# hannesweisbach/channelcoding

Measured on AMD Instinct MI355X. Metric: decoded frames/sec (coded bits/sec = value x 255), BCH(255,231) min-sum, batch=2^20, higher is better.
Workload: dtype f32

## Files before the change

### channelcoding_amd/csrc/cc_internal.hpp

```cpp
#pragma once
#include <hip/hip_runtime.h>

#include <cstdint>
#include <memory>
#include <mutex>
#include <string>
#include <vector>

#include "../../include/channelcoding_amd.h"
#include "galois.hpp"

namespace ccamd {

struct MinSumGeometry {
  int W = 64, C = 4, frames_per_wave = 1, KW = 1;
};

struct MinSumParams {
  int n, K, KW;
  int variant;
  int stop_rule;
  unsigned iterations;
  float alpha_f;
  float beta_f;
  double beta_d;
  const uint32_t *colmask;
  float *gstate;
  unsigned long long gslab;
  uint32_t *ctl = nullptr;
  unsigned sample = 0;
  uint32_t *list = nullptr;
  unsigned list_cap = 0;
  int gate = -1;
  int first_pass = 0;
  int dual = 0;
  const float *llr2 = nullptr;
  uint8_t *hard2 = nullptr;
  uint16_t *iters2 = nullptr;
  int32_t *status2 = nullptr;
};

#if defined(__HIPCC__)
__device__ __forceinline__ bool two_pass_sampled(const MinSumParams &p) { return p.ctl[2] * 8u < p.sample; }
__device__ __forceinline__ bool two_pass_in_effect(const uint32_t *ctl, unsigned sample, unsigned cap) {
  return ctl[2] * 8u < sample && ctl[3] == 0u && ctl[1] <= cap;
}
#endif

struct AlgebraicTables {
  uint8_t exp[512];
  uint8_t log[512];
  uint8_t g[256];
  uint8_t roots_log[64];
  int n, k, l, t, nroots, family, q;
};

struct WideTables {
  const uint16_t *exp = nullptr, *log = nullptr;
  const uint16_t *g = nullptr;
  uint32_t root_log[64] = {0};
  uint32_t n = 0, k = 0, l = 0, t = 0, nroots = 0, q = 0;
  int family = 0;
};

}

namespace ccamd {
struct McWorkspace;
void mc_workspace_free(McWorkspace *w);
struct HostStage;
void host_stage_free(HostStage *s);
}

struct cc_code {
  cc_desc desc;
  int device = 0;
  std::unique_ptr<ccamd::Field> field;
  ccamd::CodeTables tab;
  bool wide = false;
  std::unique_ptr<ccamd::FieldT<uint16_t>> field16;
  ccamd::CodeTablesT<uint16_t> tab16;
  ccamd::WideTables wide_dev;
  uint16_t *d_wide = nullptr;
  bool soft = false;
  std::vector<uint8_t> custom_H;
  bool matrix_only = false;
  unsigned ms_rows = 0;
  ccamd::MinSumGeometry geo;
  uint32_t *d_colmask = nullptr;
  uint16_t *d_diag = nullptr;
  uint32_t *d_colbits = nullptr;
  uint8_t *d_parity = nullptr;
  ccamd::AlgebraicTables *d_alg = nullptr;
  ccamd::AlgebraicTables h_alg;
  mutable ccamd::McWorkspace *mc = nullptr;
  mutable ccamd::HostStage *stage = nullptr;
  mutable std::mutex lazy_lock;
  hipMemPool_t pool = nullptr;
  int num_cus = 256;
  bool force_generic = false;
  std::string name;
};

namespace ccamd {

inline hipError_t workspace_alloc(const cc_code *code, void **p, size_t bytes, hipStream_t stream) {
  return code->pool ? hipMallocFromPoolAsync(p, bytes, code->pool, stream) : hipMallocAsync(p, bytes, stream);
}

void set_last_error(const std::string &s);
int hip_fail(hipError_t e, const char *what);

#define CC_HIP_TRY(expr)                                   \
  do {                                                     \
    hipError_t _e = (expr);                                \
    if (_e != hipSuccess) return ccamd::hip_fail(_e, #expr); \
  } while (0)

int launch_minsum(const cc_code *code, const float *d_llr, const uint16_t *d_er, const uint32_t *d_er_off,
                  uint8_t *d_hard, float *d_L, uint16_t *d_iters, int32_t *d_status, size_t B, hipStream_t stream);
struct DiagGeometry {
  unsigned n, k, w;
  int D, LPF, CPL;
  bool scms;
  int np = 0;
  int gap[4] = {0, 0, 0, 0};
};
const DiagGeometry *diag_geometry(const CodeTables &t);
std::vector<uint16_t> build_diag_table(const CodeTables &t, int D, int W, int np = 0, const int *gap = nullptr);
size_t minsum_diag_lds_bytes(const DiagGeometry &g);
MinSumParams minsum_params(const cc_code *code);
bool minsum_shortcuts_enabled();
bool minsum_diag_supported(const cc_code *code);
int launch_minsum_diag_compact(const cc_code *code, uint32_t *d_ctl, unsigned cap, const float *d_llr, uint8_t *d_hard,
                               uint16_t *d_iters, int32_t *d_status, hipStream_t stream);
std::string minsum_diag_name(const cc_code *code);
int launch_minsum_diag(const cc_code *code, const MinSumParams &p, const float *d_llr, const uint16_t *d_er,
                       const uint32_t *d_er_off, uint8_t *d_hard, float *d_L, uint16_t *d_iters, int32_t *d_status,
                       size_t B, hipStream_t stream);
bool algebraic_long_needed(const cc_code *code, bool erasures);
int launch_algebraic_long(const cc_code *code, bool float_in, const void *d_in, const uint16_t *d_er,
                          const uint32_t *d_er_off, uint8_t *d_out, int32_t *d_nerr, int32_t *d_status, size_t B,
                          hipStream_t stream);
int launch_algebraic(const cc_code *code, bool float_in, const void *d_in, const uint16_t *d_er,
                     const uint32_t *d_er_off, uint8_t *d_out, int32_t *d_nerr, int32_t *d_status, size_t B,
                     hipStream_t stream);
bool algebraic_chunk_supported(const cc_code *code, bool erasures);
int launch_algebraic_chunk(const cc_code *code, bool float_in, const void *d_in, const uint16_t *d_er,
                           const uint32_t *d_er_off, uint8_t *d_out, int32_t *d_nerr, int32_t *d_status, size_t B,
                           hipStream_t stream);
bool bitslice_supported(const cc_code *code);
int launch_bitslice_syndromes(const cc_code *code, bool float_in, const void *d_in, uint8_t *d_out, uint8_t *d_synd, size_t B,
                              hipStream_t stream);
bool bitslice_encode_supported(const cc_code *code);
int launch_bitslice_encode(const cc_code *code, const uint8_t *d_msg, uint8_t *d_cw, size_t B, hipStream_t stream);
int launch_pgz_erasures(const cc_code *code, const uint8_t *d_in, const uint16_t *d_er, const uint32_t *d_er_off,
                        uint8_t *d_out, int32_t *d_nerr, int32_t *d_status, size_t B, hipStream_t stream);
constexpr int diag_variant_part(int variant, int parts) {
  const int order = variant == CC_ALG_MS ? 0 : variant == CC_ALG_NMS ? 1 : variant == CC_ALG_OMS ? 2
                  : variant == CC_ALG_SCMS2 ? 3 : variant == CC_ALG_SCMS1 ? 4 : 5;
  return order % parts;
}

int launch_wide_correct(const cc_code *code, const uint16_t *d_in, const uint16_t *d_er, const uint32_t *d_off,
                        uint16_t *d_out, int32_t *d_nerr, int32_t *d_status, size_t B, hipStream_t stream);
int launch_wide_pgz_erasures(const cc_code *code, const uint16_t *d_in, const uint16_t *d_er, const uint32_t *d_off,
                        uint16_t *d_out, int32_t *d_nerr, int32_t *d_status, size_t B, hipStream_t stream);
int launch_wide_encode(const cc_code *code, const uint16_t *d_msg, uint16_t *d_cw, size_t B, hipStream_t stream);
int launch_wide_extract(const cc_code *code, const uint16_t *d_cw, uint16_t *d_msg, size_t B, hipStream_t stream);
std::vector<uint8_t> build_parity_table(const Field &f, const CodeTables &t);
int launch_encode(const cc_code *code, const uint8_t *d_msg, uint8_t *d_cw, size_t B, hipStream_t stream);
int launch_encode_bits(const cc_code *code, const uint8_t *d_msg, uint8_t *d_cw, size_t B, hipStream_t stream);
int launch_extract(const cc_code *code, const uint8_t *d_cw, uint8_t *d_msg, size_t B, hipStream_t stream);
int mc_run(cc_code *code, double ebno_db, uint64_t seed, uint64_t first_frame, size_t frames, int random_codewords,
           uint64_t *d_counters, hipStream_t stream);
int mc_awgn(cc_code *code, double ebno_db, uint64_t seed, uint64_t first_frame, size_t frames, int random_codewords,
            float *d_llr, uint8_t *d_sent, hipStream_t stream);
int minsum_kernel_info(const cc_code *code, std::string &name, uint32_t &frames_per_wg, uint32_t &threads,
                       uint32_t &lds);

}
```

### channelcoding_amd/csrc/mc.hip

```cpp
#include <cmath>
#include <mutex>

#include "cc_internal.hpp"
#include "wave_ops.hpp"

namespace ccamd {
namespace {

struct Philox {
  uint32_t c[4];
};

__device__ __forceinline__ Philox philox4x32_10(uint32_t c0, uint32_t c1, uint32_t c2, uint32_t c3, uint32_t k0,
                                                uint32_t k1) {
  constexpr uint32_t M0 = 0xD2511F53u, M1 = 0xCD9E8D57u, W0 = 0x9E3779B9u, W1 = 0xBB67AE85u;
#pragma unroll
  for (int r = 0; r < 10; ++r) {
    const uint64_t p0 = static_cast<uint64_t>(M0) * c0, p1 = static_cast<uint64_t>(M1) * c2;
    const uint32_t hi0 = static_cast<uint32_t>(p0 >> 32), lo0 = static_cast<uint32_t>(p0);
    const uint32_t hi1 = static_cast<uint32_t>(p1 >> 32), lo1 = static_cast<uint32_t>(p1);
    const uint32_t n0 = hi1 ^ c1 ^ k0, n1 = lo1, n2 = hi0 ^ c3 ^ k1, n3 = lo0;
    c0 = n0;
    c1 = n1;
    c2 = n2;
// ... 262 lines not shown

}

struct McWorkspace {
  std::mutex lock;
  size_t chunk = 0;
  float *llr = nullptr;
  uint8_t *sent = nullptr, *msg = nullptr, *hard = nullptr;
  uint16_t *iters = nullptr;
  int32_t *status = nullptr, *nerr = nullptr;
  uint32_t *list = nullptr;
  hipEvent_t done = nullptr;
  int fence_in(hipStream_t stream) {
    if (done) CC_HIP_TRY(hipStreamWaitEvent(stream, done, 0));
    return CC_OK;
  }
  int fence_out(hipStream_t stream) {
    if (!done) CC_HIP_TRY(hipEventCreateWithFlags(&done, hipEventDisableTiming));
    CC_HIP_TRY(hipEventRecord(done, stream));
    return CC_OK;
  }
  ~McWorkspace() {
    if (done) (void)hipEventDestroy(done);
    for (void *p : {static_cast<void *>(llr), static_cast<void *>(sent), static_cast<void *>(msg),
                    static_cast<void *>(hard), static_cast<void *>(iters), static_cast<void *>(status),
                    static_cast<void *>(nerr), static_cast<void *>(list)})
      if (p) (void)hipFree(p);
  }
};

void mc_workspace_free(McWorkspace *w) { delete w; }

static int ensure_workspace(cc_code *code, size_t chunk) {
  if (!code->mc) code->mc = new McWorkspace();
  McWorkspace &w = *code->mc;
  if (w.chunk >= chunk) return CC_OK;
  const size_t n = code->tab.n, l = code->tab.l;
  for (void **p : {reinterpret_cast<void **>(&w.llr), reinterpret_cast<void **>(&w.sent),
                   reinterpret_cast<void **>(&w.msg), reinterpret_cast<void **>(&w.hard),
                   reinterpret_cast<void **>(&w.iters), reinterpret_cast<void **>(&w.status),
                   reinterpret_cast<void **>(&w.nerr), reinterpret_cast<void **>(&w.list)})
    if (*p) {
      (void)hipFree(*p);
      *p = nullptr;
    }
  w.chunk = 0;
  CC_HIP_TRY(hipMalloc(reinterpret_cast<void **>(&w.llr), chunk * n * sizeof(float)));
  CC_HIP_TRY(hipMalloc(reinterpret_cast<void **>(&w.sent), chunk * n));
  CC_HIP_TRY(hipMalloc(reinterpret_cast<void **>(&w.msg), chunk * l));
  CC_HIP_TRY(hipMalloc(reinterpret_cast<void **>(&w.hard), chunk * n));
  CC_HIP_TRY(hipMalloc(reinterpret_cast<void **>(&w.iters), chunk * sizeof(uint16_t)));
  CC_HIP_TRY(hipMalloc(reinterpret_cast<void **>(&w.status), chunk * sizeof(int32_t)));
  CC_HIP_TRY(hipMalloc(reinterpret_cast<void **>(&w.nerr), chunk * sizeof(int32_t)));
  CC_HIP_TRY(hipMalloc(reinterpret_cast<void **>(&w.list), (chunk + 64) * sizeof(uint32_t)));
  w.chunk = chunk;
  return CC_OK;
}

static int launch_sent_words(const cc_code *code, uint64_t seed, uint64_t first_frame, size_t frames, uint8_t *d_sent,
                             uint8_t *d_msg_scratch, hipStream_t stream) {
  if (!d_sent || !d_msg_scratch) return CC_ERR_INVALID_ARGUMENT;
  const int l = static_cast<int>(code->tab.l);
  const uint32_t k0 = static_cast<uint32_t>(seed), k1 = static_cast<uint32_t>(seed >> 32);
  int bits_log2 = 0;
  while ((16 << bits_log2) < l) ++bits_log2;
  const unsigned long long items = static_cast<unsigned long long>(frames) << bits_log2;
  hipLaunchKernelGGL(random_bits_kernel, dim3(grid_for(code, items)), dim3(256), 0, stream, d_msg_scratch, l, bits_log2,
                     static_cast<unsigned long long>(first_frame), static_cast<unsigned long long>(frames), k0, k1);
  return launch_encode_bits(code, d_msg_scratch, d_sent, frames, stream);
}

static bool mc_precheck_pays(const cc_code *code, double ebno_db) {
  if (!code->soft || code->d_colbits == nullptr || !minsum_diag_supported(code) || code->force_generic) return false;
  if (!minsum_shortcuts_enabled()) return false;
  const unsigned n = code->tab.n;
  if (n <= 128 || n > 256) return false;
  const int alg = code->desc.algorithm;
  const bool scaled = alg == CC_ALG_NMS || alg == CC_ALG_2DNMS;
  if (scaled && !(code->desc.alpha > 0.0)) return false;
  const double sigma = cc_sigma(code, ebno_db);
  const double pbit = 0.5 * std::erfc(1.0 / (sigma * std::sqrt(2.0)));
  return std::pow(1.0 - pbit, static_cast<double>(n)) >= 0.25;
}

int launch_awgn(const cc_code *code, double ebno_db, uint64_t seed, uint64_t first_frame, size_t frames,
                int random_codewords, float *d_llr, uint8_t *d_sent, uint8_t *d_msg_scratch, hipStream_t stream,
                unsigned long long *d_counters = nullptr, bool hard_bytes = false) {
  if (frames == 0) return CC_OK;
  const int n = static_cast<int>(code->tab.n);
  const float sigma = static_cast<float>(cc_sigma(code, ebno_db));
  const uint32_t k0 = static_cast<uint32_t>(seed), k1 = static_cast<uint32_t>(seed >> 32);
  const uint8_t *sent = nullptr;
  if (random_codewords) {
    const int rc = launch_sent_words(code, seed, first_frame, frames, d_sent, d_msg_scratch, stream);
    if (rc != CC_OK) return rc;
    sent = d_sent;
  } else if (d_sent) {
    CC_HIP_TRY(hipMemsetAsync(d_sent, 0, frames * static_cast<size_t>(n), stream));
  }
  int group_log2 = 0;
  while ((4 << group_log2) < n) ++group_log2;
  const unsigned long long items = static_cast<unsigned long long>(frames) << group_log2;
  if (hard_bytes)
    hipLaunchKernelGGL(awgn_kernel<true>, dim3(grid_for(code, items)), dim3(256), 0, stream, d_llr, sent, n, group_log2,
                       static_cast<unsigned long long>(first_frame), static_cast<unsigned long long>(frames), sigma, k0,
                       k1, d_counters);
  else
    hipLaunchKernelGGL(awgn_kernel<false>, dim3(grid_for(code, items)), dim3(256), 0, stream, d_llr, sent, n, group_log2,
                       static_cast<unsigned long long>(first_frame), static_cast<unsigned long long>(frames), sigma, k0,
                       k1, d_counters);
  hipError_t e = hipGetLastError();
  if (e != hipSuccess) return hip_fail(e, "awgn kernel launch");
  return CC_OK;
}

int mc_run(cc_code *code, double ebno_db, uint64_t seed, uint64_t first_frame, size_t frames, int random_codewords,
           uint64_t *d_counters, hipStream_t stream) {
  if (frames == 0) return CC_OK;
  const size_t chunk_max = size_t(1) << 20;
  const size_t chunk = frames < chunk_max ? frames : chunk_max;
  if (!code->mc) code->mc = new McWorkspace();
  std::lock_guard<std::mutex> guard(code->mc->lock);
  int rc = ensure_workspace(code, chunk);
  if (rc != CC_OK) return rc;
  McWorkspace &w = *code->mc;
  rc = w.fence_in(stream);
  if (rc != CC_OK) return rc;
  const int n = static_cast<int>(code->tab.n);
  const bool precheck = mc_precheck_pays(code, ebno_db);
  for (size_t done = 0; done < frames; done += chunk) {
    const size_t m = frames - done < chunk ? frames - done : chunk;
    uint8_t *sent = random_codewords ? w.sent : nullptr;
    if (precheck) {
      if (random_codewords) {
        rc = launch_sent_words(code, seed, first_frame + done, m, w.sent, w.msg, stream);
        if (rc != CC_OK) return rc;
      }
      uint32_t *ctl = w.list, *list = w.list + 64;
      CC_HIP_TRY(hipMemsetAsync(ctl, 0, 64 * sizeof(uint32_t), stream));
      const float sigma = static_cast<float>(cc_sigma(code, ebno_db));
      const unsigned long long wg = (m + 31) / 32, cap = static_cast<unsigned long long>(code->num_cus) * 8;
      hipLaunchKernelGGL(awgn_precheck_kernel, dim3(static_cast<int>(wg < cap ? wg : cap)), dim3(256), 0, stream, w.llr, list,
                         ctl, sent, code->d_colbits, n, code->desc.stop_rule,
                         static_cast<unsigned long long>(first_frame + done), static_cast<unsigned long long>(m), sigma,
                         static_cast<uint32_t>(seed), static_cast<uint32_t>(seed >> 32),
                         reinterpret_cast<unsigned long long *>(d_counters));
      hipError_t e = hipGetLastError();
      if (e != hipSuccess) return hip_fail(e, "awgn pre-check kernel launch");
      rc = launch_minsum_diag_compact(code, ctl, static_cast<unsigned>(m), w.llr, w.hard, w.iters, w.status, stream);
      if (rc != CC_OK) return rc;
      const unsigned long long blocks = (m + 15) / 16, max_grid = static_cast<unsigned long long>(code->num_cus) * 8;
      hipLaunchKernelGGL(count_kernel, dim3(static_cast<int>(blocks < max_grid ? blocks : max_grid)), dim3(256), 0, stream,
                         w.hard, sent, w.iters, w.status, n, code->desc.iterations, static_cast<unsigned long long>(m),
                         reinterpret_cast<unsigned long long *>(d_counters), list, ctl + 1);
      e = hipGetLastError();
      if (e != hipSuccess) return hip_fail(e, "count kernel launch");
      continue;
    }
    rc = launch_awgn(code, ebno_db, seed, first_frame + done, m, random_codewords, w.llr, sent, w.msg, stream,
                     reinterpret_cast<unsigned long long *>(d_counters), !code->soft);
    if (rc != CC_OK) return rc;
    if (code->soft)
      rc = launch_minsum(code, w.llr, nullptr, nullptr, w.hard, nullptr, w.iters, w.status, m, stream);
    else
      rc = launch_algebraic(code, false, w.llr, nullptr, nullptr, w.hard, w.nerr, w.status, m, stream);
    if (rc != CC_OK) return rc;
    const unsigned long long blocks = (m + 15) / 16;
    const unsigned long long max_grid = static_cast<unsigned long long>(code->num_cus) * 8;
    hipLaunchKernelGGL(count_kernel, dim3(static_cast<int>(blocks < max_grid ? blocks : max_grid)), dim3(256), 0, stream,
                       w.hard, sent, code->soft ? w.iters : nullptr, w.status, n, code->desc.iterations,
                       static_cast<unsigned long long>(m), reinterpret_cast<unsigned long long *>(d_counters));
    hipError_t e = hipGetLastError();
    if (e != hipSuccess) return hip_fail(e, "count kernel launch");
  }
  return w.fence_out(stream);
}


int mc_awgn(cc_code *code, double ebno_db, uint64_t seed, uint64_t first_frame, size_t frames, int random_codewords,
            float *d_llr, uint8_t *d_sent, hipStream_t stream) {
  if (frames == 0) return CC_OK;
  if (!random_codewords) return launch_awgn(code, ebno_db, seed, first_frame, frames, 0, d_llr, d_sent, nullptr, stream);
  const size_t chunk_max = size_t(1) << 20;
  const size_t chunk = frames < chunk_max ? frames : chunk_max;
  if (!code->mc) code->mc = new McWorkspace();
  std::lock_guard<std::mutex> guard(code->mc->lock);
  int rc = ensure_workspace(code, chunk);
  if (rc != CC_OK) return rc;
  McWorkspace &w = *code->mc;
  rc = w.fence_in(stream);
  if (rc != CC_OK) return rc;
  const size_t n = code->tab.n;
  for (size_t done = 0; done < frames; done += chunk) {
    const size_t m = frames - done < chunk ? frames - done : chunk;
    uint8_t *sent = d_sent ? d_sent + done * n : w.sent;
    rc = launch_awgn(code, ebno_db, seed, first_frame + done, m, 1, d_llr + done * n, sent, w.msg, stream);
    if (rc != CC_OK) return rc;
  }
  return w.fence_out(stream);
}

}
// ... 1 lines not shown
```

### channelcoding_amd/csrc/minsum_diag.hip

```cpp
#include "minsum_diag_impl.hpp"

#include <algorithm>
#include <cstdlib>

namespace ccamd {

using DiagLaunch = int (*)(const cc_code *, const MinSumParams &, const float *, const uint16_t *, const uint32_t *,
                           uint8_t *, float *, uint16_t *, int32_t *, size_t, hipStream_t);
#define CC_PART_DECL(NAME, I)                                                                                        \
  int launch_minsum_diag_##NAME##_p##I(const cc_code *, const MinSumParams &, const float *, const uint16_t *,       \
                                       const uint32_t *, uint8_t *, float *, uint16_t *, int32_t *, size_t, hipStream_t);
#define CC_PARTS_1(M, NAME) M(NAME, 0)
#define CC_PARTS_2(M, NAME) CC_PARTS_1(M, NAME) M(NAME, 1)
#define CC_PARTS_3(M, NAME) CC_PARTS_2(M, NAME) M(NAME, 2)
#define CC_PARTS_6(M, NAME) CC_PARTS_3(M, NAME) M(NAME, 3) M(NAME, 4) M(NAME, 5)
#define GEO(NAME, N, KK, W, DD, LL, CC, OO, SC, PA, LK, PP) CC_PARTS_##PP(CC_PART_DECL, NAME)
#include "minsum_diag_geos.inc"
#undef GEO
namespace {
struct DiagEntry {
  DiagGeometry geo;
  int parts;
  DiagLaunch launch[6];
};
// ... 190 lines not shown
  if (!g) return "minsum_diag_kernel";
  return "minsum_diag_kernel<K=" + std::to_string(g->k) + ",D=" + std::to_string(g->D) + ",LPF=" +
         std::to_string(g->LPF) + ",row-pipelined>";
}

size_t minsum_diag_lds_bytes(const DiagGeometry &g) {
  const bool partial = g.w != static_cast<unsigned>(g.LPF * g.D);
  const size_t fpw = 64 / g.LPF, rc = static_cast<size_t>(g.LPF) * g.CPL + (partial ? 48 : (g.LPF == 8 && g.CPL == 8 ? 8 : 16));
  return 4 * (fpw * rc * 8 + (fpw / 2) * rc * 8) + 256 * 4 +
         4 * static_cast<size_t>(g.CPL) * 256;
}


namespace {

__global__ void __launch_bounds__(256)
twopass_gather_kernel(const uint32_t *__restrict__ ctl, unsigned sample, unsigned cap, const uint32_t *__restrict__ list,
                      const float *__restrict__ llr, float *__restrict__ llr2, int n) {
  if (!two_pass_in_effect(ctl, sample, cap)) return;
  const unsigned long long cnt = ctl[1];
  const int lane = threadIdx.x & 63;
  const unsigned long long nwaves = static_cast<unsigned long long>(gridDim.x) * 4;
  for (unsigned long long k = static_cast<unsigned long long>(blockIdx.x) * 4 + (threadIdx.x >> 6); k < cnt; k += nwaves) {
    const float *src = llr + static_cast<unsigned long long>(list[k]) * n;
    float *dst = llr2 + k * n;
    for (int j = lane; j < n; j += 64) dst[j] = src[j];
  }
}
__global__ void __launch_bounds__(256)
twopass_scatter_kernel(const uint32_t *__restrict__ ctl, unsigned sample, unsigned cap, const uint32_t *__restrict__ list,
                       const uint8_t *__restrict__ hard2, const uint16_t *__restrict__ iters2,
                       const int32_t *__restrict__ status2, uint8_t *__restrict__ hard, uint16_t *__restrict__ iters,
                       int32_t *__restrict__ status, int n) {
  if (!two_pass_in_effect(ctl, sample, cap)) return;
  const unsigned long long cnt = ctl[1];
  const int lane = threadIdx.x & 63;
  const unsigned long long nwaves = static_cast<unsigned long long>(gridDim.x) * 4;
  for (unsigned long long k = static_cast<unsigned long long>(blockIdx.x) * 4 + (threadIdx.x >> 6); k < cnt; k += nwaves) {
    const unsigned long long f = list[k];
    for (int j = lane; j < n; j += 64) hard[f * n + j] = hard2[k * n + j];
    if (lane == 0) {
      if (iters) iters[f] = iters2[k];
      if (status) status[f] = status2[k];
    }
  }
}

bool two_pass_enabled() { return minsum_shortcuts_enabled(); }

int launch_two_pass(const cc_code *code, const DiagEntry *e, const MinSumParams &p, const float *d_llr, uint8_t *d_hard,
                    uint16_t *d_iters, int32_t *d_status, size_t B, hipStream_t stream) {
  const size_t n = code->tab.n, cap = B / 4, sample = 4096;
  auto up = [](size_t v) { return (v + 255) & ~static_cast<size_t>(255); };
  const size_t o_list = 256, o_llr = o_list + up(cap * 4), o_hard = o_llr + up(cap * n * 4), o_it = o_hard + up(cap * n),
               o_st = o_it + up(cap * 2), total = o_st + up(cap * 4);
  uint8_t *ws = nullptr;
  CC_HIP_TRY(workspace_alloc(code, reinterpret_cast<void **>(&ws), total, stream));
  uint32_t *ctl = reinterpret_cast<uint32_t *>(ws), *list = reinterpret_cast<uint32_t *>(ws + o_list);
  float *llr2 = reinterpret_cast<float *>(ws + o_llr);
  uint8_t *hard2 = ws + o_hard;
  uint16_t *it2 = reinterpret_cast<uint16_t *>(ws + o_it);
  int32_t *st2 = reinterpret_cast<int32_t *>(ws + o_st);
  int rc = CC_OK;
  hipError_t he = hipMemsetAsync(ctl, 0, 256, stream);
  if (he != hipSuccess) rc = hip_fail(he, "two-pass control words");
  MinSumParams q = p;
  q.ctl = ctl;
  q.list = list;
  q.list_cap = static_cast<unsigned>(cap);
  constexpr unsigned den = 8;
  q.sample = static_cast<unsigned>(sample * 8 / den);
  q.first_pass = 2;
  const size_t runs = B >= 16 * sample ? 4 : 1, per = sample / runs, hop = (B / runs) & ~static_cast<size_t>(63);
  for (size_t r = 0; r < runs && rc == CC_OK; ++r) {
    const size_t at = r * hop;
    rc = launcher(e, q)(code, q, d_llr + at * n, nullptr, nullptr, d_hard + at * n, nullptr, d_iters ? d_iters + at : nullptr,
                        d_status ? d_status + at : nullptr, per, stream);
  }
  if (rc == CC_OK) {
    q.first_pass = 1;
    q.gate = 1;
    rc = launcher(e, q)(code, q, d_llr, nullptr, nullptr, d_hard, nullptr, d_iters, d_status, B, stream);
  }
  if (rc == CC_OK) {
    const int grid = code->num_cus * 4;
    const unsigned su = q.sample, cu = q.list_cap;
    hipLaunchKernelGGL(twopass_gather_kernel, dim3(grid), dim3(256), 0, stream, ctl, su, cu, list, d_llr, llr2,
                       static_cast<int>(n));
    q.first_pass = 0;
    q.gate = -1;
    q.dual = 1;
    q.llr2 = llr2;
    q.hard2 = hard2;
    q.iters2 = it2;
    q.status2 = st2;
    rc = launcher(e, q)(code, q, d_llr, nullptr, nullptr, d_hard, nullptr, d_iters, d_status, B, stream);
    if (rc == CC_OK)
      hipLaunchKernelGGL(twopass_scatter_kernel, dim3(grid), dim3(256), 0, stream, ctl, su, cu, list, hard2, it2, st2,
                         d_hard, d_iters, d_status, static_cast<int>(n));
  }
  if (rc == CC_OK) {
    he = hipGetLastError();
    if (he != hipSuccess) rc = hip_fail(he, "two-pass kernels launch");
  }
  (void)hipFreeAsync(ws, stream);
  return rc;
}

}

bool minsum_shortcuts_enabled() {
  static const bool v = [] {
    const char *e = std::getenv("CC_AMD_TWO_PASS");
    return !(e && e[0] == '0');
  }();
  return v;
}

int launch_minsum_diag_compact(const cc_code *code, uint32_t *d_ctl, unsigned cap, const float *d_llr, uint8_t *d_hard,
                               uint16_t *d_iters, int32_t *d_status, hipStream_t stream) {
  const DiagEntry *e = diag_entry(code->tab);
  if (!e) return CC_ERR_UNSUPPORTED;
  MinSumParams q = minsum_params(code);
  q.ctl = d_ctl;
  q.sample = 1;
  q.list_cap = cap;
  q.gate = -1;
  q.dual = 1;
  q.llr2 = d_llr;
  q.hard2 = d_hard;
  q.iters2 = d_iters;
  q.status2 = d_status;
  return launcher(e, q)(code, q, d_llr, nullptr, nullptr, d_hard, nullptr, d_iters, d_status, cap, stream);
}

int launch_minsum_diag(const cc_code *code, const MinSumParams &p, const float *d_llr, const uint16_t *d_er,
                       const uint32_t *d_er_off, uint8_t *d_hard, float *d_L, uint16_t *d_iters, int32_t *d_status,
                       size_t B, hipStream_t stream) {
  const DiagEntry *e = diag_entry(code->tab);
  if (!e) return CC_ERR_UNSUPPORTED;
  const bool plain = p.variant == CC_ALG_MS || p.variant == CC_ALG_NMS || p.variant == CC_ALG_OMS || p.variant == CC_ALG_2DNMS;
  const double work = static_cast<double>(B) * code->tab.n * code->tab.k;
  if (two_pass_enabled() && plain && p.stop_rule != CC_STOP_AS_SHIPPED && p.iterations >= 2 && d_er_off == nullptr &&
      d_L == nullptr && work >= 1.5e9)
    return launch_two_pass(code, e, p, d_llr, d_hard, d_iters, d_status, B, stream);
  return launcher(e, p)(code, p, d_llr, d_er, d_er_off, d_hard, d_L, d_iters, d_status, B, stream);
}

}
```

### channelcoding_amd/csrc/minsum_diag_impl.hpp

```cpp
#pragma once
#include <cstdio>
#include <cstdlib>
#include <type_traits>
#include <utility>

#include "cc_internal.hpp"
#include "wave_ops.hpp"


namespace ccamd {
namespace {



template <int... Is, typename F>
__device__ __forceinline__ void static_for_impl(std::integer_sequence<int, Is...>, F &&f) {
  (f(std::integral_constant<int, Is>{}), ...);
}
template <int N, typename F>
__device__ __forceinline__ void static_for(F &&f) {
  static_for_impl(std::make_integer_sequence<int, N>{}, static_cast<F &&>(f));
}
template <int... Gs>
struct PairGaps {
// ... 168 lines not shown
    const int so = signum(q_old);
    return (so == 0 || so == signum(tmp)) ? tmp : 0.0f;
  } else {
    return (tmp * q_old > 0.0f) ? tmp : 0.5f * (tmp + q_old);
  }
}

template <int VARIANT>
__device__ __forceinline__ float horizontal(float m, float alpha_f, double beta_d) {
  if constexpr (VARIANT == CC_ALG_NMS || VARIANT == CC_ALG_2DNMS) {
    return __fmul_rn(alpha_f, m);
  } else if constexpr (VARIANT == CC_ALG_OMS) {
    const double a = static_cast<double>(m) - beta_d;
    return static_cast<float>((a < 0.0) ? 0.0 : a);
  } else {
    return m;
  }
}

template <int K, int D, int VARIANT, int RB, int LPF, int CPL, int OCC, bool PARTIAL, typename PG = PairGaps<>,
          bool SINGLE = false, bool CHAIN = false>
__global__ void __launch_bounds__(256, OCC)
minsum_diag_kernel(MinSumParams p, const uint16_t *__restrict__ diag_s, const uint32_t *__restrict__ colbits,
                   const float *__restrict__ llr, const uint16_t *__restrict__ er, const uint32_t *__restrict__ er_off,
                   uint8_t *__restrict__ hard, float *__restrict__ Lout, uint16_t *__restrict__ iters_out,
                   int32_t *__restrict__ status_out, unsigned long long B) {
  static_assert(K % RB == 0 && K <= 32, "row batching");
  if (p.gate == 1 && !two_pass_sampled(p)) return;
  if (p.dual && two_pass_in_effect(p.ctl, p.sample, p.list_cap)) {
    llr = p.llr2;
    hard = p.hard2;
    Lout = nullptr;
    iters_out = p.iters2;
    status_out = p.status2;
    B = p.ctl[1] < p.list_cap ? p.ctl[1] : p.list_cap;
  }
  static_assert(LPF == 8 || LPF == 16, "a frame occupies half or all of a 16-lane DPP row");
  static_assert(2 * PG::NP <= D && !(PARTIAL && PG::NP > 0), "paired slots");
  static_assert(!CHAIN || PG::NP == 0 || (PG::gap(0) == 1 && PG::gap(PG::NP - 1) == 1), "links are gap-1 pairs");
  constexpr int NLK = CHAIN ? PG::NP : 0;
  constexpr int FPW = 64 / LPF;
  constexpr int RC = LPF * CPL + (PARTIAL ? 48 : (LPF == 8 && CPL == 8 ? 8 : 16));
  extern __shared__ __attribute__((aligned(16))) char smem[];
  constexpr int CY_BYTES = FPW * RC * 8, CN_BYTES = (FPW / 2) * RC * 8;
  constexpr int WAVE_BYTES = CY_BYTES + (SINGLE ? 0 : CN_BYTES);
  const int lane = threadIdx.x & 63, wid = threadIdx.x >> 6;
  const int fl = lane / LPF, lam = lane & (LPF - 1);
  char *cy_base = smem + wid * WAVE_BYTES;
  char *cn_lane = cy_base + CY_BYTES + ((fl >> 1) - fl) * RC * 8 + (fl & 1) * 4;
  uint32_t *cbits = reinterpret_cast<uint32_t *>(smem + 4 * WAVE_BYTES);
  char *stg = smem + 4 * WAVE_BYTES + 1024 + wid * (CPL * 256);
  const uint32_t stg_lds = __builtin_amdgcn_readfirstlane(static_cast<uint32_t>(reinterpret_cast<size_t>(stg)));
  cbits[threadIdx.x] = colbits[threadIdx.x];
  __shared__ unsigned wg_next;
  if (threadIdx.x == 0) wg_next = 2 * 4 * (64 / LPF);
  __syncthreads();

  const int n = p.n;
  int aCY[D];
#pragma unroll
  for (int d = 0; d < D; ++d) aCY[d] = (fl * RC + diag_s[d * LPF + lam]) * 8;
  float pen = 0.0f;
  uint32_t sgn_keep = 0xFFFFFFFFu;
  if constexpr (PARTIAL) {
    if (diag_s[(D - 1) * LPF + lam] == 0xFFFFu) {
      aCY[D - 1] = (fl * RC + LPF * CPL + 16) * 8;
      pen = 3.402823466e+38f;
      sgn_keep = 0u;
    }
  }
  const int col0 = fl * RC + lam;
  const bool oddf = SINGLE && (fl & 1);
#ifndef CC_EXP_O0_B32
  auto cell_y = [&](float2 v) -> float { return SINGLE ? (oddf ? v.x : v.y) : v.y; };
  auto cell_cs = [&](float2 v) -> float { return SINGLE ? (oddf ? v.y : v.x) : v.x; };
#else
  auto cell_y = [&](float2 v) -> float { return v.y; };
  auto cell_cs = [&](float2 v) -> float { return v.x; };
#endif
  auto make_cell = [&](float cs, float y) -> float2 { return (SINGLE && oddf) ? make_float2(y, cs) : make_float2(cs, y); };
  const int y_off = (SINGLE && oddf) ? 0 : 4;
  int aWR[SINGLE ? D : 1];
  if constexpr (SINGLE) {
#pragma unroll
    for (int d = 0; d < D; ++d) aWR[d] = aCY[d] + (oddf ? 4 : 0);
  }

  const unsigned long long ngroups = static_cast<unsigned long long>(gridDim.x) * 4 * FPW;
  constexpr unsigned GPW = 4 * FPW;
  auto ordinal_frame = [&](unsigned o) -> unsigned long long {
    return static_cast<unsigned long long>(blockIdx.x) * GPW + (o % GPW) + static_cast<unsigned long long>(o / GPW) * ngroups;
  };
  auto take_frame = [&]() -> unsigned long long {
    unsigned o = 0;
    if (lam == 0) o = atomicAdd(&wg_next, 1u);
    o = static_cast<unsigned>(__builtin_amdgcn_ds_bpermute((lane & ~(LPF - 1)) * 4, static_cast<int>(o)));
    return ordinal_frame(o);
  };
  unsigned long long frame = (static_cast<unsigned long long>(blockIdx.x) * 4 + wid) * FPW + fl;
  unsigned long long nextf = frame + ngroups;
  bool active = frame < B;
  unsigned it = 0;
  constexpr bool NEEDQ = (VARIANT == CC_ALG_SCMS1 || VARIANT == CC_ALG_SCMS2);
  constexpr bool QONLY = !SINGLE && ((VARIANT == CC_ALG_SCMS2 && 2 * K * D + 64 > 256) ||
                                     (VARIANT == CC_ALG_SCMS1 && K * D >= 160 && OCC >= 2));
  constexpr bool KEEPQ = (VARIANT == CC_ALG_SCMS2 && !SINGLE) || QONLY;
  float R[(SINGLE || QONLY) ? 1 : K][(SINGLE || QONLY) ? 1 : D];
  float Q[KEEPQ ? K : 1][KEEPQ ? D : 1];
  __shared__ uint2 row_state[QONLY ? 4 * FPW * K : 1];
  uint2 *const my_rows = row_state + (QONLY ? (wid * FPW + fl) * K : 0);
  uint2 rsq = make_uint2(0u, 0u);
  constexpr bool BITS1 = VARIANT == CC_ALG_SCMS1 && !SINGLE && !QONLY;
  constexpr int RPW = 32 / D;
  constexpr int NW = (K + RPW - 1) / RPW;
  uint32_t SW[BITS1 ? NW : 1], ZW[BITS1 ? NW : 1];

  constexpr bool X4 = (LPF * CPL - 1) >= 4 * LPF;
  constexpr int NF = (LPF * CPL - 1) / (4 * LPF);
  auto stage = [&](unsigned long long f) {
    if (f < B) {
      const float *src = llr + f * n;
      if constexpr (X4) {
        const float *v = src + 4 * lam;
        const float *vt = v + (n - 4 * LPF);
        uint32_t m0_save;
        const uint32_t sb = __builtin_amdgcn_readfirstlane(stg_lds);
        static_assert(NF == 1 || NF == 3, "x4 staging is written out for one or three aligned copies");
        if constexpr (NF == 3) {
          asm volatile(
              "s_mov_b32 %0, m0\n\ts_mov_b32 m0, %3\n\ts_nop 0\n\tglobal_load_lds_dwordx4 %1, off\n\t"
              "s_add_u32 m0, %3, %4\n\ts_nop 0\n\tglobal_load_lds_dwordx4 %1, off offset:%7\n\t"
              "s_add_u32 m0, %3, %5\n\ts_nop 0\n\tglobal_load_lds_dwordx4 %1, off offset:%8\n\t"
              "s_add_u32 m0, %3, %6\n\ts_nop 0\n\tglobal_load_lds_dwordx4 %2, off\n\ts_mov_b32 m0, %0"
              : "=&s"(m0_save)
              : "v"(v), "v"(vt), "s"(sb), "n"(1024 - LPF * 16), "n"(2048 - 2 * LPF * 16), "n"(3072), "n"(LPF * 16),
                "n"(2 * LPF * 16)
              : "memory", "scc");
        } else {
          asm volatile(
              "s_mov_b32 %0, m0\n\ts_mov_b32 m0, %3\n\ts_nop 0\n\tglobal_load_lds_dwordx4 %1, off\n\t"
              "s_add_u32 m0, %3, 1024\n\ts_nop 0\n\tglobal_load_lds_dwordx4 %2, off\n\ts_mov_b32 m0, %0"
              : "=&s"(m0_save)
              : "v"(v), "v"(vt), "s"(sb)
              : "memory", "scc");
        }
      } else {
#pragma unroll
        for (int c = 0; c < CPL; ++c) {
          const int j = lam + LPF * c;
          if (j < n) {
            uint32_t m0_save;
            asm volatile("s_mov_b32 %0, m0\n\ts_mov_b32 m0, %2\n\ts_nop 0\n\tglobal_load_lds_dword %1, off\n\ts_mov_b32 m0, %0"
                         : "=&s"(m0_save) : "v"(src + j), "s"(stg_lds + c * 256) : "memory");
          }
        }
      }
    }
  };
  const char *stg_full = stg + fl * LPF * 16 + lam * 4;
  const char *stg_tail = stg + NF * 1024 + fl * LPF * 16 + (lam - n + 4 * LPF) * 4;
  auto staged = [&](int c) -> float {
    if constexpr (X4) {
      if (c < 4 * NF) return *reinterpret_cast<const float *>(stg_full + (c / 4) * 1024 + (c % 4) * 4 * LPF);
      return *reinterpret_cast<const float *>(stg_tail + 4 * LPF * c);
    } else {
      return *reinterpret_cast<const float *>(stg + c * 256 + lane * 4);
    }
  };
  auto setup = [&](unsigned long long f) {
#pragma unroll
    for (int c = 0; c < CPL; ++c) {
      float y = staged(c) + 0.0f;
      if (c == CPL - 1 && lam + LPF * c >= n) y = 0.0f;
      *reinterpret_cast<float2 *>(cy_base + (col0 + LPF * c) * 8) = make_cell(0.0f, y);
    }
    if (er_off != nullptr) {
      for (uint32_t e = er_off[f]; e < er_off[f + 1]; ++e) {
        const int pos = er[e];
        if ((pos & (LPF - 1)) == lam) *reinterpret_cast<float *>(cy_base + (fl * RC + pos) * 8 + y_off) = 0.0f;
      }
    }
    if constexpr (!SINGLE && !QONLY) static_for<K>([&](auto I) { static_for<D>([&](auto Dd) { R[I][Dd] = 0.0f; }); });
    if constexpr (KEEPQ) static_for<K>([&](auto I) { static_for<D>([&](auto Dd) { Q[I][Dd] = 0.0f; }); });
    if constexpr (QONLY)
      for (int r = lam; r < K; r += LPF) my_rows[r] = make_uint2(0u, 0u);
    if constexpr (BITS1) static_for<NW>([&](auto Wd) { SW[Wd] = 0u; ZW[Wd] = 0xFFFFFFFFu; });
  };

#pragma unroll
  for (int c = 0; c < CPL; ++c)
    if constexpr (!SINGLE) *reinterpret_cast<float *>(cn_lane + (col0 + LPF * c) * 8) = 0.0f;
  if (active) {
    stage(frame);
    asm volatile("s_waitcnt vmcnt(0)" ::: "memory");
    setup(frame);
    stage(nextf);
  }

  while (__any(active)) {
    constexpr bool PREFETCH = !(BITS1 && K * D >= 160) && !SINGLE;
#ifdef CC_EXP_TRED
    constexpr bool TRED = LPF == 16 && K % 4 == 0 && !SINGLE;
#else
    constexpr bool TRED = false;
#endif
    constexpr bool EARLY_PF = TRED && PREFETCH;
    float2 cyq[D];
    float2 carry_cy[NLK ? NLK : 1];
    float carry_sum[NLK ? NLK : 1];
    auto fetch = [&](auto IC) {
      constexpr int row = decltype(IC)::value;
      if constexpr (QONLY) rsq = my_rows[row];
      static_for<D>([&](auto DD) {
        constexpr int d = DD;
        if constexpr (d < 2 * NLK && (d & 1) == 0 && row >= 1) {
          cyq[d] = carry_cy[d / 2];
          return;
        }
#ifdef CC_EXP_NO_CYR
        asm volatile("" : "=v"(cyq[d].x), "=v"(cyq[d].y));
#else
#ifdef CC_EXP_O0_B32
        if constexpr (SINGLE) {
          const int at = aCY[slot_base<PG>(d)] + 8 * (row + slot_gap<PG>(d));
          cyq[d].x = *reinterpret_cast<const float *>(cy_base + at + (4 - y_off));
          cyq[d].y = *reinterpret_cast<const float *>(cy_base + at + y_off);
          return;
        }
#endif
        cyq[d] = *reinterpret_cast<const float2 *>(cy_base + aCY[slot_base<PG>(d)] + 8 * (row + slot_gap<PG>(d)));
#endif
      });
    };
    float Tloc[D];
    auto row_front = [&](auto IR, uint32_t &o1, uint32_t &o2, uint32_t &os) {
      constexpr int i = decltype(IR)::value;
      if constexpr (!PREFETCH) fetch(IR);
      [[maybe_unused]] auto wget = [&](auto DD) -> float {
        if constexpr (SINGLE) return Tloc[DD];
        else if constexpr (QONLY) return Q[i][DD];
        else return R[i][DD];
      };
      auto wset = [&](auto DD, float v) {
        if constexpr (SINGLE) Tloc[DD] = v;
        else if constexpr (!QONLY) R[i][DD] = v;
      };
      [[maybe_unused]] const float old_hi = u2f(rsq.y & 0x7FFFFFFFu);
      [[maybe_unused]] uint32_t old_Y = (rsq.x ^ rsq.y);
      if constexpr (QONLY) asm volatile("" : "+v"(old_Y));
// ... 207 lines not shown
#endif
        row_back(IR, m1[0], m2[0], sg[0], cn);
      });
    }

    uint32_t acc = 0;
    auto stop_scan = [&](auto ORC) {
      float cnv[CPL], yc[CPL];
      uint32_t cb[CPL];
#pragma unroll
      for (int c = 0; c < CPL; ++c) {
        if constexpr (SINGLE) {
          const float2 cy = *reinterpret_cast<const float2 *>(cy_base + (col0 + LPF * c) * 8);
          cnv[c] = cy.x;
          yc[c] = cy.y;
        } else {
          cnv[c] = *reinterpret_cast<const float *>(cn_lane + (col0 + LPF * c) * 8);
          yc[c] = *reinterpret_cast<const float *>(cy_base + (col0 + LPF * c) * 8 + 4);
        }
        cb[c] = cbits[lam + LPF * c];
      }
      asm volatile("" ::: "memory");
#pragma unroll
      for (int c = 0; c < CPL; ++c) {
        const int m = static_cast<int>(f2u(cnv[c] + yc[c])) >> 31;
        if constexpr (decltype(ORC)::value)
          acc = static_cast<uint32_t>(__builtin_amdgcn_bitop3_b32(static_cast<int>(acc), m, static_cast<int>(cb[c]), 0xF8));
        else
          acc = static_cast<uint32_t>(__builtin_amdgcn_bitop3_b32(static_cast<int>(acc), m, static_cast<int>(cb[c]), 0x78));
      }
      if constexpr (!SINGLE) {
#pragma unroll
        for (int c = 0; c < CPL; ++c) {
          *reinterpret_cast<float *>(cy_base + (col0 + LPF * c) * 8) = cnv[c];
          *reinterpret_cast<float *>(cn_lane + (col0 + LPF * c) * 8) = 0.0f;
        }
      }
    };
    bool ok;
    if (SINGLE && p.stop_rule == CC_STOP_AS_SHIPPED) {
      ok = true;
    } else if (p.stop_rule == CC_STOP_PUBLISHED) {
      stop_scan(std::true_type{});
      ok = group_or<LPF>(acc) == 0;
    } else {
      stop_scan(std::false_type{});
      ok = (p.stop_rule == CC_STOP_AS_SHIPPED) || group_xor<LPF>(acc) == 0;
    }
#ifdef CC_EXP_NEVER_STOP
    ok = false;
#endif
    const bool finished = SINGLE || ok || (it + 1 >= p.iterations);
    if (finished && active) {
      const unsigned long long done = frame;
      const unsigned done_it = ok ? it : p.iterations;
      frame = nextf;
      active = frame < B;
      uint8_t *hp = hard + done * n + lam;
      float *Lp = Lout ? Lout + done * n + lam : nullptr;
      const bool handed = SINGLE && p.first_pass != 0 && !ok;
      auto emit = [&](int c, float L) {
        if (handed) return;
        if (c < CPL - 1 || lam + LPF * c < n) {
          hp[LPF * c] = (L < 0.0f) ? 1 : 0;
          if (Lp) Lp[LPF * c] = L;
        }
      };
      if (active) {
        asm volatile("s_waitcnt vmcnt(0)" ::: "memory");
#pragma unroll
        for (int c = 0; c < CPL; ++c) {
          const float2 cy = *reinterpret_cast<const float2 *>(cy_base + (col0 + LPF * c) * 8);
          float y = staged(c) + 0.0f;
          if (c == CPL - 1 && lam + LPF * c >= n) y = 0.0f;
          *reinterpret_cast<float2 *>(cy_base + (col0 + LPF * c) * 8) = make_cell(0.0f, y);
          emit(c, cy.x + cy.y);
        }
        if (er_off != nullptr) {
          for (uint32_t e = er_off[frame]; e < er_off[frame + 1]; ++e) {
            const int pos = er[e];
            if ((pos & (LPF - 1)) == lam) *reinterpret_cast<float *>(cy_base + (fl * RC + pos) * 8 + y_off) = 0.0f;
          }
        }
        if constexpr (!SINGLE && !QONLY) static_for<K>([&](auto I) { static_for<D>([&](auto Dd) { R[I][Dd] = 0.0f; }); });
        if constexpr (KEEPQ) static_for<K>([&](auto I) { static_for<D>([&](auto Dd) { Q[I][Dd] = 0.0f; }); });
        if constexpr (QONLY)
          for (int r = lam; r < K; r += LPF) my_rows[r] = make_uint2(0u, 0u);
        if constexpr (BITS1) static_for<NW>([&](auto Wd) { SW[Wd] = 0u; ZW[Wd] = 0xFFFFFFFFu; });
        it = 0;
      } else {
#pragma unroll
        for (int c = 0; c < CPL; ++c) {
          const float2 cy = *reinterpret_cast<const float2 *>(cy_base + (col0 + LPF * c) * 8);
          emit(c, cy.x + cy.y);
        }
      }
      if (lam == 0) {
        if (handed) {
          if (p.first_pass == 2) {
            atomicAdd(&p.ctl[2], 1u);
          } else {
            const uint32_t at = atomicAdd(&p.ctl[1], 1u);
            if (at < p.list_cap) p.list[at] = static_cast<uint32_t>(done);
            else p.ctl[3] = 1u;
          }
        } else {
          if (iters_out) iters_out[done] = static_cast<uint16_t>(done_it);
          if (status_out) status_out[done] = ok ? CC_FRAME_OK : CC_FRAME_NOT_CONVERGED;
        }
      }
      if (active) {
        nextf = take_frame();
        stage(nextf);
      }
    } else {
      ++it;
    }
  }
  asm volatile("s_waitcnt vmcnt(0)" ::: "memory");
}

}

namespace {

template <int K, int D, int LPF, int CPL, int OCC, bool SCMS = false, bool PARTIAL = false, typename PG = PairGaps<>,
          bool CHAIN = false, int PARTS = 1, int PART = 0>
int launch_diag_geometry(const cc_code *code, const MinSumParams &p, const float *d_llr, const uint16_t *d_er,
                         const uint32_t *d_er_off, uint8_t *d_hard, float *d_L, uint16_t *d_iters, int32_t *d_status,
                         size_t B, hipStream_t stream) {
  constexpr int RB = 1;
  constexpr bool Q_ONLY_2 = 2 * K * D + 64 > 256, Q_ONLY_1 = K * D >= 160 && OCC >= 2;
  constexpr int OCC_S = Q_ONLY_2 ? OCC : (2 * K * D + 64 <= 128) ? 4 : (2 * K * D + 64 <= 168) ? 3 : 2;
  constexpr int FPW = 64 / LPF;
  if (!(code->tab.n > static_cast<unsigned>(LPF * (CPL - 1)) && code->tab.n <= static_cast<unsigned>(LPF * CPL))) {
    set_last_error("minsum_diag: only the last owned column of a lane may lie beyond the frame");
    return CC_ERR_UNSUPPORTED;
  }
  const DiagGeometry g{0, 0, PARTIAL ? 1u : static_cast<unsigned>(LPF * D), D, LPF, CPL, SCMS};
  const size_t lds = minsum_diag_lds_bytes(g);
  const unsigned long long blocks_needed = (B + 4 * FPW - 1) / (4 * FPW);
  unsigned long long per_cu = (160 * 1024) / lds;
  const unsigned long long occ = p.variant == CC_ALG_SCMS2 ? static_cast<unsigned long long>(OCC_S) : OCC;
  if ((p.variant == CC_ALG_SCMS2 && Q_ONLY_2) || (p.variant == CC_ALG_SCMS1 && Q_ONLY_1))
    per_cu = (160 * 1024) / (lds + 4 * FPW * K * sizeof(uint2));
  if (per_cu > occ) per_cu = occ;
  const unsigned long long max_grid = static_cast<unsigned long long>(code->num_cus) * per_cu;
  const int grid = static_cast<int>(blocks_needed < max_grid ? blocks_needed : max_grid);
  const unsigned long long Bq = B;
  hipError_t e = hipSuccess;
  const bool single = p.stop_rule == CC_STOP_AS_SHIPPED || p.iterations == 1 || p.first_pass != 0;
  constexpr size_t rc_cols = static_cast<size_t>(LPF) * CPL + (PARTIAL ? 48 : (LPF == 8 && CPL == 8 ? 8 : 16));
  const size_t lds_s = lds - 4 * (FPW / 2) * rc_cols * 8;
  unsigned long long per_cu_s = (160 * 1024) / lds_s;
  if (per_cu_s > 8) per_cu_s = 8;
  const unsigned long long max_grid_s = static_cast<unsigned long long>(code->num_cus) * per_cu_s;
  const int grid_s = static_cast<int>(blocks_needed < max_grid_s ? blocks_needed : max_grid_s);
#define CC_LAUNCH_S(V, O, S)                                                                                       \
  {                                                                                                                \
    const size_t lds_k = (S) ? lds_s : lds;                                                                        \
    const int grid_k = (S) ? grid_s : grid;                                                                        \
    e = hipFuncSetAttribute(                                                                                       \
        reinterpret_cast<const void *>(&minsum_diag_kernel<K, D, V, RB, LPF, CPL, O, PARTIAL, PG, S, CHAIN>),      \
        hipFuncAttributeMaxDynamicSharedMemorySize, static_cast<int>(lds_k));                                     \
    if (e == hipSuccess)                                                                                           \
      hipLaunchKernelGGL((minsum_diag_kernel<K, D, V, RB, LPF, CPL, O, PARTIAL, PG, S, CHAIN>), dim3(grid_k), dim3(256), lds_k, \
                         stream, p, code->d_diag, code->d_colbits, d_llr, d_er, d_er_off, d_hard, d_L, d_iters,    \
                         d_status, Bq);                                                                            \
  }
#define CC_LAUNCH(V, O)                                                                                            \
  {                                                                                                                \
    if constexpr (diag_variant_part(V, PARTS) != PART) e = hipErrorInvalidValue;                                   \
    else if (single) CC_LAUNCH_S(V, OCC, true) else CC_LAUNCH_S(V, O, false)                                       \
  }
  switch (p.variant) {
    case CC_ALG_MS: CC_LAUNCH(CC_ALG_MS, OCC) break;
    case CC_ALG_NMS: CC_LAUNCH(CC_ALG_NMS, OCC) break;
    case CC_ALG_OMS: CC_LAUNCH(CC_ALG_OMS, OCC) break;
    case CC_ALG_2DNMS: CC_LAUNCH(CC_ALG_2DNMS, OCC) break;
    case CC_ALG_SCMS1:
      CC_LAUNCH(CC_ALG_SCMS1, OCC)
      break;
    case CC_ALG_SCMS2:
      if constexpr (SCMS) CC_LAUNCH(CC_ALG_SCMS2, OCC_S) else e = hipErrorInvalidValue;
      break;
    default: e = hipErrorInvalidValue;
  }
#undef CC_LAUNCH
#undef CC_LAUNCH_S
  if (e == hipSuccess) e = hipGetLastError();
  if (e != hipSuccess) return hip_fail(e, "minsum_diag kernel launch");
  return CC_OK;
}

}

}
```

Before: 61.81 million.

## Shard the dynamic frame-claim counter across 32 pool lines with ordinal draws

Replaces the single workgroup-shared frame counter scheme with a global pool of 32 sharded atomic counters, each on its own cache line. Each frame group draws its next frame ordinal from its shard, optionally one frame ahead, and keeps the current and next ordinals in LDS. The aim is to cut contention on work-stealing atomics and balance load across early-terminating frames. In exchange it adds workspace allocation and a memset per launch, extra LDS that can lower occupancy, and a hard limit of 2^32 frames per call.

Result: faster. 68.12 million (median of 6 runs) (+10.2%).

```diff
diff --git a/channelcoding_amd/csrc/cc_internal.hpp b/channelcoding_amd/csrc/cc_internal.hpp
--- a/channelcoding_amd/csrc/cc_internal.hpp
+++ b/channelcoding_amd/csrc/cc_internal.hpp
@@ -28,6 +28,7 @@
   float *gstate;
   unsigned long long gslab;
   uint32_t *ctl = nullptr;
+  uint32_t *pool = nullptr;
   unsigned sample = 0;
   uint32_t *list = nullptr;
   unsigned list_cap = 0;
@@ -39,6 +40,9 @@
   uint16_t *iters2 = nullptr;
   int32_t *status2 = nullptr;
 };
+
+constexpr unsigned POOL_SHARDS = 32;
+constexpr size_t POOL_WORDS = POOL_SHARDS * 32;
 
 #if defined(__HIPCC__)
 __device__ __forceinline__ bool two_pass_sampled(const MinSumParams &p) { return p.ctl[2] * 8u < p.sample; }
@@ -132,8 +136,8 @@
 MinSumParams minsum_params(const cc_code *code);
 bool minsum_shortcuts_enabled();
 bool minsum_diag_supported(const cc_code *code);
-int launch_minsum_diag_compact(const cc_code *code, uint32_t *d_ctl, unsigned cap, const float *d_llr, uint8_t *d_hard,
-                               uint16_t *d_iters, int32_t *d_status, hipStream_t stream);
+int launch_minsum_diag_compact(const cc_code *code, uint32_t *d_ctl, uint32_t *d_pool, unsigned cap, const float *d_llr,
+                               uint8_t *d_hard, uint16_t *d_iters, int32_t *d_status, hipStream_t stream);
 std::string minsum_diag_name(const cc_code *code);
 int launch_minsum_diag(const cc_code *code, const MinSumParams &p, const float *d_llr, const uint16_t *d_er,
                        const uint32_t *d_er_off, uint8_t *d_hard, float *d_L, uint16_t *d_iters, int32_t *d_status,
diff --git a/channelcoding_amd/csrc/mc.hip b/channelcoding_amd/csrc/mc.hip
--- a/channelcoding_amd/csrc/mc.hip
+++ b/channelcoding_amd/csrc/mc.hip
@@ -338,7 +338,7 @@
   CC_HIP_TRY(hipMalloc(reinterpret_cast<void **>(&w.iters), chunk * sizeof(uint16_t)));
   CC_HIP_TRY(hipMalloc(reinterpret_cast<void **>(&w.status), chunk * sizeof(int32_t)));
   CC_HIP_TRY(hipMalloc(reinterpret_cast<void **>(&w.nerr), chunk * sizeof(int32_t)));
-  CC_HIP_TRY(hipMalloc(reinterpret_cast<void **>(&w.list), (chunk + 64) * sizeof(uint32_t)));
+  CC_HIP_TRY(hipMalloc(reinterpret_cast<void **>(&w.list), (chunk + 64 + POOL_WORDS) * sizeof(uint32_t)));
   w.chunk = chunk;
   return CC_OK;
 }
@@ -422,8 +422,8 @@
         rc = launch_sent_words(code, seed, first_frame + done, m, w.sent, w.msg, stream);
         if (rc != CC_OK) return rc;
       }
-      uint32_t *ctl = w.list, *list = w.list + 64;
-      CC_HIP_TRY(hipMemsetAsync(ctl, 0, 64 * sizeof(uint32_t), stream));
+      uint32_t *ctl = w.list, *pool = w.list + 64, *list = w.list + 64 + POOL_WORDS;
+      CC_HIP_TRY(hipMemsetAsync(ctl, 0, (64 + POOL_WORDS) * sizeof(uint32_t), stream));
       const float sigma = static_cast<float>(cc_sigma(code, ebno_db));
       const unsigned long long wg = (m + 31) / 32, cap = static_cast<unsigned long long>(code->num_cus) * 8;
       hipLaunchKernelGGL(awgn_precheck_kernel, dim3(static_cast<int>(wg < cap ? wg : cap)), dim3(256), 0, stream, w.llr, list,
@@ -433,7 +433,7 @@
                          reinterpret_cast<unsigned long long *>(d_counters));
       hipError_t e = hipGetLastError();
       if (e != hipSuccess) return hip_fail(e, "awgn pre-check kernel launch");
-      rc = launch_minsum_diag_compact(code, ctl, static_cast<unsigned>(m), w.llr, w.hard, w.iters, w.status, stream);
+      rc = launch_minsum_diag_compact(code, ctl, pool, static_cast<unsigned>(m), w.llr, w.hard, w.iters, w.status, stream);
       if (rc != CC_OK) return rc;
       const unsigned long long blocks = (m + 15) / 16, max_grid = static_cast<unsigned long long>(code->num_cus) * 8;
       hipLaunchKernelGGL(count_kernel, dim3(static_cast<int>(blocks < max_grid ? blocks : max_grid)), dim3(256), 0, stream,
diff --git a/channelcoding_amd/csrc/minsum_diag.hip b/channelcoding_amd/csrc/minsum_diag.hip
--- a/channelcoding_amd/csrc/minsum_diag.hip
+++ b/channelcoding_amd/csrc/minsum_diag.hip
@@ -266,8 +266,9 @@
                     uint16_t *d_iters, int32_t *d_status, size_t B, hipStream_t stream) {
   const size_t n = code->tab.n, cap = B / 4, sample = 4096;
   auto up = [](size_t v) { return (v + 255) & ~static_cast<size_t>(255); };
-  const size_t o_list = 256, o_llr = o_list + up(cap * 4), o_hard = o_llr + up(cap * n * 4), o_it = o_hard + up(cap * n),
-               o_st = o_it + up(cap * 2), total = o_st + up(cap * 4);
+  constexpr size_t max_runs = 4, o_pool = 256, pool_bytes = POOL_WORDS * 4;
+  const size_t o_list = o_pool + (max_runs + 2) * pool_bytes, o_llr = o_list + up(cap * 4), o_hard = o_llr + up(cap * n * 4),
+               o_it = o_hard + up(cap * n), o_st = o_it + up(cap * 2), total = o_st + up(cap * 4);
   uint8_t *ws = nullptr;
   CC_HIP_TRY(workspace_alloc(code, reinterpret_cast<void **>(&ws), total, stream));
   uint32_t *ctl = reinterpret_cast<uint32_t *>(ws), *list = reinterpret_cast<uint32_t *>(ws + o_list);
@@ -276,7 +277,7 @@
   uint16_t *it2 = reinterpret_cast<uint16_t *>(ws + o_it);
   int32_t *st2 = reinterpret_cast<int32_t *>(ws + o_st);
   int rc = CC_OK;
-  hipError_t he = hipMemsetAsync(ctl, 0, 256, stream);
+  hipError_t he = hipMemsetAsync(ctl, 0, o_list, stream);
   if (he != hipSuccess) rc = hip_fail(he, "two-pass control words");
   MinSumParams q = p;
   q.ctl = ctl;
@@ -285,15 +286,17 @@
   constexpr unsigned den = 8;
   q.sample = static_cast<unsigned>(sample * 8 / den);
   q.first_pass = 2;
-  const size_t runs = B >= 16 * sample ? 4 : 1, per = sample / runs, hop = (B / runs) & ~static_cast<size_t>(63);
+  const size_t runs = B >= 16 * sample ? max_runs : 1, per = sample / runs, hop = (B / runs) & ~static_cast<size_t>(63);
   for (size_t r = 0; r < runs && rc == CC_OK; ++r) {
     const size_t at = r * hop;
+    q.pool = reinterpret_cast<uint32_t *>(ws + o_pool + r * pool_bytes);
     rc = launcher(e, q)(code, q, d_llr + at * n, nullptr, nullptr, d_hard + at * n, nullptr, d_iters ? d_iters + at : nullptr,
                         d_status ? d_status + at : nullptr, per, stream);
   }
   if (rc == CC_OK) {
     q.first_pass = 1;
     q.gate = 1;
+    q.pool = reinterpret_cast<uint32_t *>(ws + o_pool + max_runs * pool_bytes);
     rc = launcher(e, q)(code, q, d_llr, nullptr, nullptr, d_hard, nullptr, d_iters, d_status, B, stream);
   }
   if (rc == CC_OK) {
@@ -304,6 +307,7 @@
     q.first_pass = 0;
     q.gate = -1;
     q.dual = 1;
+    q.pool = reinterpret_cast<uint32_t *>(ws + o_pool + (max_runs + 1) * pool_bytes);
     q.llr2 = llr2;
     q.hard2 = hard2;
     q.iters2 = it2;
@@ -331,12 +335,13 @@
   return v;
 }
 
-int launch_minsum_diag_compact(const cc_code *code, uint32_t *d_ctl, unsigned cap, const float *d_llr, uint8_t *d_hard,
-                               uint16_t *d_iters, int32_t *d_status, hipStream_t stream) {
+int launch_minsum_diag_compact(const cc_code *code, uint32_t *d_ctl, uint32_t *d_pool, unsigned cap, const float *d_llr,
+                               uint8_t *d_hard, uint16_t *d_iters, int32_t *d_status, hipStream_t stream) {
   const DiagEntry *e = diag_entry(code->tab);
   if (!e) return CC_ERR_UNSUPPORTED;
   MinSumParams q = minsum_params(code);
   q.ctl = d_ctl;
+  q.pool = d_pool;
   q.sample = 1;
   q.list_cap = cap;
   q.gate = -1;
@@ -358,7 +363,16 @@
   if (two_pass_enabled() && plain && p.stop_rule != CC_STOP_AS_SHIPPED && p.iterations >= 2 && d_er_off == nullptr &&
       d_L == nullptr && work >= 1.5e9)
     return launch_two_pass(code, e, p, d_llr, d_hard, d_iters, d_status, B, stream);
-  return launcher(e, p)(code, p, d_llr, d_er, d_er_off, d_hard, d_L, d_iters, d_status, B, stream);
-}
-
-}
+  uint32_t *pool = nullptr;
+  CC_HIP_TRY(workspace_alloc(code, reinterpret_cast<void **>(&pool), POOL_WORDS * 4, stream));
+  int rc = CC_OK;
+  const hipError_t he = hipMemsetAsync(pool, 0, POOL_WORDS * 4, stream);
+  if (he != hipSuccess) rc = hip_fail(he, "frame pool");
+  MinSumParams q = p;
+  q.pool = pool;
+  if (rc == CC_OK) rc = launcher(e, q)(code, q, d_llr, d_er, d_er_off, d_hard, d_L, d_iters, d_status, B, stream);
+  (void)hipFreeAsync(pool, stream);
+  return rc;
+}
+
+}
diff --git a/channelcoding_amd/csrc/minsum_diag_impl.hpp b/channelcoding_amd/csrc/minsum_diag_impl.hpp
--- a/channelcoding_amd/csrc/minsum_diag_impl.hpp
+++ b/channelcoding_amd/csrc/minsum_diag_impl.hpp
@@ -244,8 +244,9 @@
   char *stg = smem + 4 * WAVE_BYTES + 1024 + wid * (CPL * 256);
   const uint32_t stg_lds = __builtin_amdgcn_readfirstlane(static_cast<uint32_t>(reinterpret_cast<size_t>(stg)));
   cbits[threadIdx.x] = colbits[threadIdx.x];
+  constexpr bool POOL = !SINGLE && LPF == 16;
   __shared__ unsigned wg_next;
-  if (threadIdx.x == 0) wg_next = 2 * 4 * (64 / LPF);
+  if (!POOL && threadIdx.x == 0) wg_next = 2 * 4 * (64 / LPF);
   __syncthreads();
 
   const int n = p.n;
@@ -278,8 +279,23 @@
     for (int d = 0; d < D; ++d) aWR[d] = aCY[d] + (oddf ? 4 : 0);
   }
 
-  const unsigned long long ngroups = static_cast<unsigned long long>(gridDim.x) * 4 * FPW;
   constexpr unsigned GPW = 4 * FPW;
+  const unsigned S = gridDim.x < POOL_SHARDS ? gridDim.x : POOL_SHARDS, shard = blockIdx.x % S, Ws = (gridDim.x - shard + S - 1) / S;
+  const unsigned obase = 2 * Ws * GPW;
+  auto frame_of = [&](unsigned o) -> unsigned long long { return static_cast<unsigned long long>(o) * S + shard; };
+  auto draw = [&]() -> unsigned {
+    uint32_t line = shard * 32;
+    asm volatile("" : "+v"(line));
+    return atomicAdd(p.pool + line, 1u);
+  };
+  auto drawn = [&](unsigned o) -> unsigned {
+    return obase + static_cast<unsigned>(__builtin_amdgcn_ds_bpermute((lane & ~(LPF - 1)) * 4, static_cast<int>(o)));
+  };
+  __shared__ uint2 ords[POOL ? GPW : 1];
+  uint2 &my_ords = ords[POOL ? wid * FPW + fl : 0];
+  unsigned opd = 0;
+  constexpr bool PREDRAW = !(VARIANT == CC_ALG_SCMS1 && K * D < 160);
+  const unsigned long long ngroups = static_cast<unsigned long long>(gridDim.x) * GPW;
   auto ordinal_frame = [&](unsigned o) -> unsigned long long {
     return static_cast<unsigned long long>(blockIdx.x) * GPW + (o % GPW) + static_cast<unsigned long long>(o / GPW) * ngroups;
   };
@@ -289,8 +305,16 @@
     o = static_cast<unsigned>(__builtin_amdgcn_ds_bpermute((lane & ~(LPF - 1)) * 4, static_cast<int>(o)));
     return ordinal_frame(o);
   };
-  unsigned long long frame = (static_cast<unsigned long long>(blockIdx.x) * 4 + wid) * FPW + fl;
-  unsigned long long nextf = frame + ngroups;
+  unsigned long long frame, nextf;
+  if constexpr (POOL) {
+    const unsigned ofr = (blockIdx.x / S) * GPW + wid * FPW + fl;
+    if (lam == 0) my_ords = make_uint2(ofr, ofr + Ws * GPW);
+    frame = frame_of(ofr);
+    nextf = frame_of(ofr + Ws * GPW);
+  } else {
+    frame = (static_cast<unsigned long long>(blockIdx.x) * 4 + wid) * FPW + fl;
+    nextf = frame + ngroups;
+  }
   bool active = frame < B;
   unsigned it = 0;
   constexpr bool NEEDQ = (VARIANT == CC_ALG_SCMS1 || VARIANT == CC_ALG_SCMS2);
@@ -387,6 +411,7 @@
     asm volatile("s_waitcnt vmcnt(0)" ::: "memory");
     setup(frame);
     stage(nextf);
+    if (POOL && PREDRAW && lam == 0) opd = draw();
   }
 
   while (__any(active)) {
@@ -700,9 +725,10 @@
 #endif
     const bool finished = SINGLE || ok || (it + 1 >= p.iterations);
     if (finished && active) {
-      const unsigned long long done = frame;
+      const uint2 od = POOL ? my_ords : make_uint2(0u, 0u);
+      const unsigned long long done = POOL ? frame_of(od.x) : frame;
       const unsigned done_it = ok ? it : p.iterations;
-      frame = nextf;
+      frame = POOL ? frame_of(od.y) : nextf;
       active = frame < B;
       uint8_t *hp = hard + done * n + lam;
       float *Lp = Lout ? Lout + done * n + lam : nullptr;
@@ -758,8 +784,18 @@
         }
       }
       if (active) {
-        nextf = take_frame();
-        stage(nextf);
+        if constexpr (POOL) {
+          if (!PREDRAW && lam == 0) opd = draw();
+          const unsigned nx = drawn(opd);
+          stage(frame_of(nx));
+          if (lam == 0) {
+            my_ords = make_uint2(od.y, nx);
+            if (PREDRAW) opd = draw();
+          }
+        } else {
+          nextf = take_frame();
+          stage(nextf);
+        }
       }
     } else {
       ++it;
@@ -785,13 +821,18 @@
     set_last_error("minsum_diag: only the last owned column of a lane may lie beyond the frame");
     return CC_ERR_UNSUPPORTED;
   }
+  if (p.pool == nullptr || B >= (1ull << 32)) {
+    set_last_error("minsum_diag: no frame pool, or more than 2^32 frames in one call");
+    return CC_ERR_UNSUPPORTED;
+  }
   const DiagGeometry g{0, 0, PARTIAL ? 1u : static_cast<unsigned>(LPF * D), D, LPF, CPL, SCMS};
   const size_t lds = minsum_diag_lds_bytes(g);
   const unsigned long long blocks_needed = (B + 4 * FPW - 1) / (4 * FPW);
-  unsigned long long per_cu = (160 * 1024) / lds;
+  constexpr size_t ords_bytes = LPF == 16 ? 4 * FPW * sizeof(uint2) : 0;
+  unsigned long long per_cu = (160 * 1024) / (lds + ords_bytes);
   const unsigned long long occ = p.variant == CC_ALG_SCMS2 ? static_cast<unsigned long long>(OCC_S) : OCC;
   if ((p.variant == CC_ALG_SCMS2 && Q_ONLY_2) || (p.variant == CC_ALG_SCMS1 && Q_ONLY_1))
-    per_cu = (160 * 1024) / (lds + 4 * FPW * K * sizeof(uint2));
+    per_cu = (160 * 1024) / (lds + ords_bytes + 4 * FPW * K * sizeof(uint2));
   if (per_cu > occ) per_cu = occ;
   const unsigned long long max_grid = static_cast<unsigned long long>(code->num_cus) * per_cu;
   const int grid = static_cast<int>(blocks_needed < max_grid ? blocks_needed : max_grid);
```
